# agsiddhant/PBML_Mantle_Convection

Hardware: AMD Instinct MI355X
Metric: training samples/sec (2-D 506x506 Stokes fields) (higher is better)
Workload: dtype f16+bf16; 1 GPU; CFG-3: symmetric U-Net (levels 5, c_h 16, k 5, repeats 3, reflect) + L1 data loss + divergence + Stokes momentum residual, 506x506, per-GPU batch 32, Adam, HIP-graph replay; global_batch=32, parallelism=dp1

## Files before the change

pbml_mantle_convection_amd/build_ext.py:

```python
import os
import subprocess
import sys

HERE = os.path.dirname(os.path.abspath(__file__))
CSRC = os.path.join(HERE, "csrc")
LIB = os.path.join(HERE, "libmantle_hip.so")
SOURCES = ["elementwise.hip", "conv_api.hip", "conv_f32.hip", "conv_bf16.hip", "conv_rr_bf16.hip", "loss.hip", "optim.hip"]
HEADERS = ["common.h", "conv_common.h", "conv_rr.h", os.path.join("..", "..", "include", "mantle_hip.h")]
FLAGS = ["-O3", "--offload-arch=gfx950", "-fPIC", "-std=c++17", "-Wall", "-Wno-unused-function",
         "-ffp-contract=off"]


EXTRA_FLAGS = {"conv_rr_bf16.hip": ["-fno-slp-vectorize"]}


def _stale(target, deps):
    if not os.path.exists(target):
        return True
    t = os.path.getmtime(target)
    return any(os.path.getmtime(d) > t for d in deps)


def build(force=False, verbose=True):
    hipcc = os.environ.get("HIPCC", "/opt/rocm/bin/hipcc")
    hdrs = [os.path.join(CSRC, h) for h in HEADERS]
    objdir = os.path.join(HERE, "build")
    os.makedirs(objdir, exist_ok=True)
    objs = []
    procs = []
    for src in SOURCES:
        s = os.path.join(CSRC, src)
        o = os.path.join(objdir, src.replace(".hip", ".o"))
        objs.append(o)
        if force or _stale(o, [s] + hdrs):
            cmd = [hipcc, *FLAGS, *EXTRA_FLAGS.get(src, []), "-c", s, "-o", o]
            if verbose:
                print(" ".join(cmd), flush=True)
            procs.append((src, subprocess.Popen(cmd)))
    for src, p in procs:
        if p.wait() != 0:
            raise RuntimeError(f"hipcc failed on {src}")
    if force or procs or _stale(LIB, objs):
        cmd = [hipcc, "--offload-arch=gfx950", "-shared", "-fPIC", *objs, "-o", LIB]
        if verbose:
            print(" ".join(cmd), flush=True)
        subprocess.check_call(cmd)
    return LIB


if __name__ == "__main__":
    build(force="--force" in sys.argv)
    print(LIB)
```

pbml_mantle_convection_amd/csrc/conv_api.hip:

```cpp
#include "conv_rr.h"

int mc_conv2d_f32(const ConvGeom& g, const void* x0, const void* x1, const void* bank, const float* bias, void* y0,
                  void* y1, float* part, const ConvFuse& fz, int fuse, hipStream_t s);
int mc_wgrad_f32(const ConvGeom& g, const void* x0, const void* x1, const void* dy, void* part, const ConvFuse& fz, int fuse,
                 hipStream_t s);
int mc_bf16_tile(const mc_conv_desc* d, int* th, int* tw);
size_t mc_bf16_bank_bytes(const ConvGeom& g, int dgrad);
int mc_bf16_pack(const ConvGeom& g, const float* w_unique, int dgrad, void* packed, hipStream_t s);
int mc_conv2d_bf16(const ConvGeom& g, const void* x0, const void* x1, const void* bank, const float* bias, void* y0,
                   void* y1, float* part, const ConvFuse& fz, int fuse, hipStream_t s);
int mc_wgrad_bf16(const ConvGeom& g, const void* x0, const void* x1, const void* dy, void* part, const ConvFuse& fz, int fuse,
                  hipStream_t s);
const char* mc_bf16_kernel_name(const ConvGeom& g);
void mc_bf16_bank_dims(const ConvGeom& g, int dgrad, int& chunks, int& steps, int& ntiles);
bool mc_rr_applies(int dtype, int cout, int wo, bool full_pad);
size_t mc_rr_bank_bytes(const ConvGeom& g, int dgrad);
int mc_rr_pack(const ConvGeom& g, const float* w_unique, int dgrad, void* packed, hipStream_t s);
int mc_conv2d_rr(const ConvGeom& g, const void* x0, const void* x1, const void* bank, const float* bias, void* y0, void* y1,
                 float* part, const ConvFuse& fz, int fuse, hipStream_t s);
const char* mc_rr_kernel_name(const ConvGeom& g, int fuse);

namespace {

bool rr_desc(const mc_conv_desc* d) {
  return mc_rr_applies(d->dtype, d->c_out, d->w + 2 * d->pad - d->k + 1, d->pad == d->k - 1);
}

int geom_for(const mc_conv_desc* d, ConvGeom& g) {
  if (!d) return MC_EINVAL;
  int th = 16, tw = 16;
  if (mc_is16(d->dtype)) {
    if (rr_desc(d)) { th = RR_R; tw = RR_TW; }
    else {
      int rc = mc_bf16_tile(d, &th, &tw);
      if (rc) return rc;
    }
  } else if (d->dtype != MC_F32) {
    return MC_EUNSUPPORTED;
  }
  return conv_geom(d, th, tw, g);
}
int stat_slots(const mc_conv_desc* d, const ConvGeom& g) { return rr_desc(d) ? g.tiles * RR_STRIPS : g.tiles; }

__global__ void k_pack_f32(ConvGeom g, const float* __restrict__ wu, int dgrad, float* __restrict__ bank, size_t total) {
  for (size_t i = blockIdx.x * (size_t)blockDim.x + threadIdx.x; i < total; i += (size_t)gridDim.x * blockDim.x)
    bank[i] = pack_value_f32(g, wu, i, dgrad);
}

struct PkJob {
  int K, Cout, CBin, CB0, Cin0, Cin1, Cin, U, nh, nv, nq, CBout, CinP, CoutP;
  int dgrad, steps, ntiles, bf16, f16, rr, first_block;
  unsigned total;
  const float* w;
  void* out;
};
constexpr int PK_MAX = 24;
struct PkTable { int n; PkJob j[PK_MAX]; };

__global__ void k_pack_batched(PkTable t) {
  int ji = 0;
#pragma unroll 1
  for (int k = 1; k < t.n; ++k) if ((int)blockIdx.x >= t.j[k].first_block) ji = k;
  const PkJob& job = t.j[ji];
  const int nblk = (ji + 1 < t.n ? t.j[ji + 1].first_block : (int)gridDim.x) - job.first_block;
  for (size_t i = (size_t)(blockIdx.x - job.first_block) * blockDim.x + threadIdx.x; i < job.total; i += (size_t)nblk * blockDim.x) {
    if (job.rr || job.bf16) {
      const float v = job.rr ? rr_pack_value(job, job.w, i, job.dgrad, job.ntiles)
                             : pack_value_bf16(job, job.w, i, job.dgrad, job.steps, job.ntiles);
      reinterpret_cast<bf16_t*>(job.out)[i] = job.f16 ? __builtin_bit_cast(bf16_t, (_Float16)v) : f2bf(v);
    } else {
      reinterpret_cast<float*>(job.out)[i] = pack_value_f32(job, job.w, i, job.dgrad);
    }
  }
}

struct WfJob {
  int K, U, nh, nv, nq, Cin, Cin0, CB0, CinP, CoutP, Cout, G, first_block;
  const float* part;
  float* dw;
  float* db;
};
constexpr int WF_MAX = 32;
struct WfTable { int n; WfJob j[WF_MAX]; };

constexpr int WF_WAVES = 16;
__device__ __forceinline__ void wgrad_finalize_block(const WfJob& g, int lblock) {
  const int K = g.K, KK = K * K;
  const int nch = wg_chunks(g.CinP);
  const size_t slab = wg_slab_floats(g.CoutP, g.CinP, KK);
  const size_t nW = (size_t)KK * nch * g.U * 16;
  const size_t total = nW + g.Cout;
  const int e = threadIdx.x & 63, w = threadIdx.x >> 6, NWV = (int)blockDim.x >> 6;
  const size_t i = (size_t)lblock * 64 + e;
  __shared__ float red[WF_WAVES][64];
  float s = 0.f;
  long dst = -1;
  if (i < total) {
    size_t o1, ox[3] = {0, 0, 0};
    int nx = 0;
    bool live = true;
    if (i < nW) {
      int cl = (int)(i & 15);
      size_t r = i >> 4;
      int u = (int)(r % g.U); r /= g.U;
      int chunk = (int)(r % nch);
      int tap = (int)(r / nch);
      int cip = chunk * 16 + cl;
      int ci = cip < g.CB0 * 8 ? cip : g.Cin0 + (cip - g.CB0 * 8);
      live = cip < g.CB0 * 8 ? cip < g.Cin0 : ci < g.Cin;
      int ky = tap / K, kx = tap - ky * K;
      o1 = wg_index(tap, cip, u, g.CoutP, nch);
      const int tfx = ky * K + (K - 1 - kx), tfy = (K - 1 - ky) * K + kx, tfxy = (K - 1 - ky) * K + (K - 1 - kx);
      if (u < g.nh) { nx = 1; ox[0] = wg_index(tfx, cip, g.U + u, g.CoutP, nch); }
      else if (u < g.nh + g.nv) { nx = 1; ox[0] = wg_index(tfy, cip, g.U + u, g.CoutP, nch); }
      else if (u < g.nh + g.nv + g.nq) {
        const int c0 = g.U + g.nh + g.nv + (u - g.nh - g.nv);
        nx = 3;
        ox[0] = wg_index(tfx, cip, c0, g.CoutP, nch); ox[1] = wg_index(tfy, cip, c0 + g.nq, g.CoutP, nch);
        ox[2] = wg_index(tfxy, cip, c0 + 2 * g.nq, g.CoutP, nch);
      }
      dst = ((long)u * g.Cin + ci) * KK + tap;
    } else {
      o1 = (size_t)KK * nch * g.CoutP * 16 + (i - nW);
      dst = -2 - (long)(i - nW);
    }
    if (live) {
      const float* part = g.part;
      float a0 = 0.f, a1 = 0.f, a2 = 0.f, a3 = 0.f;
      int G = w;
      for (; G + 3 * NWV < g.G; G += 4 * NWV) {
        a0 += part[(size_t)G * slab + o1]; a1 += part[(size_t)(G + NWV) * slab + o1];
        a2 += part[(size_t)(G + 2 * NWV) * slab + o1]; a3 += part[(size_t)(G + 3 * NWV) * slab + o1];
        for (int m = 0; m < nx; ++m) {
          a0 += part[(size_t)G * slab + ox[m]]; a1 += part[(size_t)(G + NWV) * slab + ox[m]];
          a2 += part[(size_t)(G + 2 * NWV) * slab + ox[m]]; a3 += part[(size_t)(G + 3 * NWV) * slab + ox[m]];
        }
      }
      for (; G < g.G; G += NWV) {
        a0 += part[(size_t)G * slab + o1];
        for (int m = 0; m < nx; ++m) a0 += part[(size_t)G * slab + ox[m]];
      }
      s = (a0 + a1) + (a2 + a3);
    } else {
      dst = -1;
    }
  }
  red[w][e] = s;
  __syncthreads();
  if (w == 0 && dst != -1) {
    float r = 0.f;
    for (int k = 0; k < NWV; k += 4) r += (red[k][e] + red[k + 1][e]) + (red[k + 2][e] + red[k + 3][e]);
    if (dst >= 0) { if (g.dw) g.dw[dst] += r; }
    else if (g.db) g.db[-2 - dst] += r;
  }
}

__global__ __launch_bounds__(64 * WF_WAVES) void k_wgrad_finalize(WfTable t) {
  int ji = 0;
#pragma unroll 1
  for (int k = 1; k < t.n; ++k) if ((int)blockIdx.x >= t.j[k].first_block) ji = k;
  wgrad_finalize_block(t.j[ji], blockIdx.x - t.j[ji].first_block);
}

int wf_fill(const mc_conv_desc* d, const void* partials, float* dw, float* db, WfJob& j, int& blocks) {
  ConvGeom g;
  int rc = geom_for(d, g);
  if (rc) return rc;
  if (!partials || (!dw && !db)) return MC_EINVAL;
  j.K = g.K; j.U = g.U; j.Cin = g.Cin; j.Cin0 = g.Cin0; j.CB0 = g.CB0; j.CinP = g.CinP; j.CoutP = g.CoutP; j.Cout = g.Cout;
  j.nh = g.nh; j.nv = g.nv; j.nq = g.nq; j.G = g.wgrad_G; j.part = (const float*)partials; j.dw = dw; j.db = db;
  size_t total = (size_t)g.K * g.K * wg_chunks(g.CinP) * g.U * 16 + g.Cout;
  blocks = (int)((total + 63) / 64);
  return MC_OK;
}

}

static bool bank_is_rr(const ConvGeom& g, int dgrad) {
  return dgrad ? mc_rr_applies(g.dtype, g.Cin, g.W + 2 * g.pad, true) : mc_rr_applies(g.dtype, g.Cout, g.Wo, g.pad == g.K - 1);
}

extern "C" {

int mc_version(void) { return 200; }

const char* mc_strerror(int code) {
  switch (code) {
    case MC_OK: return "ok";
    case MC_EINVAL: return "invalid argument or shape";
    case MC_EUNSUPPORTED: return "unsupported configuration";
    case MC_EWORKSPACE: return "workspace too small";
    default: return code > 0 ? hipGetErrorString((hipError_t)code) : "unknown error";
  }
}

size_t mc_packed_weight_bytes(const mc_conv_desc* d, int32_t dgrad) {
  ConvGeom g;
  if (geom_for(d, g)) return 0;
  if (bank_is_rr(g, dgrad)) return mc_rr_bank_bytes(g, dgrad);
  if (mc_is16(g.dtype)) return mc_bf16_bank_bytes(g, dgrad);
  int cbin = dgrad ? g.CBout : g.CBin, cop = dgrad ? g.CinP : g.CoutP;
  return (size_t)cbin * g.K * g.K * 8 * cop * sizeof(float);
}

int mc_pack_weights(const mc_conv_desc* d, const float* w_unique, int32_t dgrad, void* packed, void* stream) {
  ConvGeom g;
  int rc = geom_for(d, g);
  if (rc) return rc;
  if (!w_unique || !packed) return MC_EINVAL;
  if (bank_is_rr(g, dgrad)) return mc_rr_pack(g, w_unique, dgrad, packed, (hipStream_t)stream);
  if (mc_is16(g.dtype)) return mc_bf16_pack(g, w_unique, dgrad, packed, (hipStream_t)stream);
  size_t total = mc_packed_weight_bytes(d, dgrad) / sizeof(float);
  int blocks = (int)((total + 255) / 256);
  if (blocks > 2048) blocks = 2048;
  hipLaunchKernelGGL(k_pack_f32, dim3(blocks), dim3(256), 0, (hipStream_t)stream, g, w_unique, dgrad, (float*)packed, total);
  MC_CHECK_LAUNCH();
  return MC_OK;
}

const char* mc_conv_kernel_name(const mc_conv_desc* d) {
  ConvGeom g;
  if (geom_for(d, g)) return "unsupported";
  if (rr_desc(d)) return mc_rr_kernel_name(g, 0);
  if (mc_is16(g.dtype)) return mc_bf16_kernel_name(g);
  return g.K == 5 ? "k_conv_direct_f32<5>" : "k_conv_direct_f32<3>";
}

int32_t mc_conv_tiles(const mc_conv_desc* d) {
  ConvGeom g;
  if (geom_for(d, g)) return -1;
  return stat_slots(d, g);
}

static bool act_ok(int a) { return a >= MC_ACT_NONE && a <= MC_ACT_ELU; }

static int fill_prologue(const mc_conv_prologue* pro, ConvFuse& fz, int& rc) {
  rc = MC_OK;
  if (!pro) return 0;
  if (!act_ok(pro->act0) || !act_ok(pro->act1)) { rc = MC_EINVAL; return 0; }
  fz.coef0 = pro->coef0; fz.coef1 = pro->coef1; fz.act0 = pro->act0; fz.act1 = pro->act1;
  return (pro->coef0 || pro->coef1 || pro->act0 != MC_ACT_NONE || pro->act1 != MC_ACT_NONE) ? 1 : 0;
}

int mc_conv2d_fused(const mc_conv_desc* d, const void* x0, const void* x1, const mc_conv_prologue* pro,
                    const void* packed_w, const float* bias, void* y0, void* y1, float* stat_partials,
                    const mc_conv_epilogue* epi, void* stream) {
  ConvGeom g;
  int rc = geom_for(d, g);
  if (rc) return rc;
  if (!x0 || !packed_w || !y0 || (g.Cin1 > 0 && !x1) || (g.split8 > 0 && !y1)) return MC_EINVAL;
  ConvFuse fz = conv_fuse_none();
  int fuse = fill_prologue(pro, fz, rc);
  if (rc) return rc;
  if (epi) {
    if (fuse) return MC_EUNSUPPORTED;
    if (!epi->y || !epi->partials || !act_ok(epi->act) || epi->pad < 0 || epi->hs <= 0 || epi->ws <= 0) return MC_EINVAL;
    if (epi->pad_mode < MC_PAD_ZEROS || epi->pad_mode > MC_PAD_REFLECT) return MC_EINVAL;
    if (g.split8 > 0 || stat_partials || g.out_f32) return MC_EUNSUPPORTED;
    if (g.Ho != epi->hs + 2 * epi->pad || g.Wo != epi->ws + 2 * epi->pad) return MC_EINVAL;
    fz.ey = epi->y; fz.ecoef = epi->coef; fz.epart = epi->partials; fz.eact = epi->act; fz.epad = epi->pad;
    fz.ezero = epi->pad_mode == MC_PAD_ZEROS || epi->pad == 0; fz.ehs = epi->hs; fz.ews = epi->ws;
    if (epi->y_f16 && g.dtype != MC_BF16) return MC_EINVAL;
    fz.ey16 = epi->y_f16 ? 1 : 0;
    if (epi->part_stride < stat_slots(d, g)) return MC_EINVAL;
    fz.estride = epi->part_stride;
    fuse = 2;
  }
  if (rr_desc(d)) return mc_conv2d_rr(g, x0, x1, packed_w, bias, y0, y1, stat_partials, fz, fuse, (hipStream_t)stream);
  if (mc_is16(g.dtype)) return mc_conv2d_bf16(g, x0, x1, packed_w, bias, y0, y1, stat_partials, fz, fuse, (hipStream_t)stream);
  return mc_conv2d_f32(g, x0, x1, packed_w, bias, y0, y1, stat_partials, fz, fuse, (hipStream_t)stream);
}

int mc_conv2d(const mc_conv_desc* d, const void* x0, const void* x1, const void* packed_w, const float* bias, void* y0,
              void* y1, float* stat_partials, void* stream) {
  return mc_conv2d_fused(d, x0, x1, nullptr, packed_w, bias, y0, y1, stat_partials, nullptr, stream);
}

size_t mc_conv_bank_read_extent(const mc_conv_desc* d) {
  ConvGeom g;
  if (geom_for(d, g)) return 0;
  const int KK = g.K * g.K;
  if (rr_desc(d)) {
    const size_t nfrag = g.K == 5 ? RR<5>::NFRAG : RR<3>::NFRAG;
    const size_t chunks = (g.CBin + 1) / 2, groups = (g.Cout + 15) / 16;
    return (((chunks - 1) * groups + (groups - 1)) * nfrag * 64 + (nfrag * 64 - 1)) * 16 + 16;
  }
  if (mc_is16(g.dtype)) {
    int chunks, steps, ntiles;
    mc_bf16_bank_dims(g, 0, chunks, steps, ntiles);
    const size_t last = ((size_t)(chunks - 1) * steps + (steps - 1)) * ntiles + (ntiles - 1);
    return (last * 64 + 63) * 16 + 16;
  }
  const int ncog = (g.CoutP + 15) / 16, co0 = 16 * (ncog - 1);
  const int comax = g.CoutP - 1 - co0;
  const size_t last = (((size_t)(g.CBin - 1) * KK + (KK - 1)) * 8 + 7) * g.CoutP + co0 + (comax >= 15 ? 15 : comax);
  return (last + 1) * sizeof(float);
}

size_t mc_wgrad_partial_bytes(const mc_conv_desc* d) {
  ConvGeom g;
  if (geom_for(d, g)) return 0;
  return (size_t)g.wgrad_G * wg_slab_floats(g.CoutP, g.CinP, g.K * g.K) * sizeof(float);
}

int mc_conv2d_wgrad_fused(const mc_conv_desc* d, const void* x0, const void* x1, const mc_conv_prologue* pro,
                          const void* dy, void* partials, void* stream) {
  ConvGeom g;
  int rc = geom_for(d, g);
  if (rc) return rc;
  if (!x0 || !dy || !partials || (g.Cin1 > 0 && !x1)) return MC_EINVAL;
  ConvFuse fz = conv_fuse_none();
  const int fuse = fill_prologue(pro, fz, rc);
  if (rc) return rc;
  if (mc_is16(g.dtype)) return mc_wgrad_bf16(g, x0, x1, dy, partials, fz, fuse, (hipStream_t)stream);
  return mc_wgrad_f32(g, x0, x1, dy, partials, fz, fuse, (hipStream_t)stream);
}

int mc_conv2d_wgrad(const mc_conv_desc* d, const void* x0, const void* x1, const void* dy, void* partials,
                    void* stream) {
  return mc_conv2d_wgrad_fused(d, x0, x1, nullptr, dy, partials, stream);
}

int mc_conv2d_wgrad_finalize_batched(const mc_conv_desc* descs, const void* const* partials, float* const* dw,
                                     float* const* db, int32_t n, void* stream) {
  if (!descs || !partials || !dw || !db || n <= 0) return MC_EINVAL;
  for (int pass = 0; pass < 2; ++pass) {
    WfTable t;
    t.n = 0;
    int blocks = 0;
    auto flush = [&]() {
      if (t.n == 0) return;
      hipLaunchKernelGGL(k_wgrad_finalize, dim3(blocks), dim3(pass == 0 ? 64 * WF_WAVES : 256), 0, (hipStream_t)stream, t);
      t.n = 0; blocks = 0;
    };
    for (int k = 0; k < n; ++k) {
      WfJob j;
      int b = 0;
      int rc = wf_fill(&descs[k], partials[k], dw[k], db[k], j, b);
      if (rc) return rc;
      if ((j.G >= 128) != (pass == 0)) continue;
      j.first_block = blocks;
      t.j[t.n++] = j;
      blocks += b;
      if (t.n == WF_MAX) flush();
    }
    flush();
    MC_CHECK_LAUNCH();
  }
  return MC_OK;
}

int mc_conv2d_wgrad_finalize(const mc_conv_desc* d, const void* partials, float* dw_unique, float* dbias,
                             void* stream) {
  return mc_conv2d_wgrad_finalize_batched(d, &partials, &dw_unique, &dbias, 1, stream);
}

int mc_pack_weights_batched(const mc_conv_desc* descs, const float* const* w_unique, const int32_t* dgrad,
                            void* const* packed, int32_t n, void* stream) {
  if (!descs || !w_unique || !dgrad || !packed || n <= 0) return MC_EINVAL;
  for (int base = 0; base < n; base += PK_MAX) {
    PkTable t;
    t.n = n - base < PK_MAX ? n - base : PK_MAX;
    int blocks = 0;
    for (int k = 0; k < t.n; ++k) {
      ConvGeom g;
      int rc = geom_for(&descs[base + k], g);
      if (rc) return rc;
      if (!w_unique[base + k] || !packed[base + k]) return MC_EINVAL;
      PkJob& j = t.j[k];
      j.K = g.K; j.Cout = g.Cout; j.CBin = g.CBin; j.CB0 = g.CB0; j.Cin0 = g.Cin0; j.Cin1 = g.Cin1; j.Cin = g.Cin; j.U = g.U;
      j.nh = g.nh; j.nv = g.nv; j.nq = g.nq;
      j.CBout = g.CBout; j.CinP = g.CinP; j.CoutP = g.CoutP; j.dgrad = dgrad[base + k]; j.bf16 = mc_is16(g.dtype);
      j.f16 = (g.dtype == MC_MIX16 && !j.dgrad) ? 1 : 0;
      j.rr = bank_is_rr(g, j.dgrad);
      size_t total;
      if (j.rr) {
        j.steps = 0;
        j.ntiles = ((j.dgrad ? g.CinP : g.Cout) + 15) / 16;
        total = mc_rr_bank_bytes(g, j.dgrad) / 2;
      } else if (j.bf16) {
        int chunks;
        mc_bf16_bank_dims(g, j.dgrad, chunks, j.steps, j.ntiles);
        total = (size_t)chunks * j.steps * j.ntiles * 64 * 8;
      } else {
        j.steps = 0; j.ntiles = 0;
        total = (size_t)(j.dgrad ? g.CBout : g.CBin) * g.K * g.K * 8 * (j.dgrad ? g.CinP : g.CoutP);
      }
      j.total = (unsigned)total;
      j.w = w_unique[base + k];
      j.out = packed[base + k];
      j.first_block = blocks;
      int b = (int)((total + 256 * 8 - 1) / (256 * 8));
      blocks += b < 1 ? 1 : b;
    }
    hipLaunchKernelGGL(k_pack_batched, dim3(blocks), dim3(256), 0, (hipStream_t)stream, t);
    MC_CHECK_LAUNCH();
  }
  return MC_OK;
}

}
```

Measured before the change: 3235 samples/s.

## Add flat-plane MFMA conv kernel for deep low-resolution 5x5 bf16/f16 layers

Adds a new persistent MFMA convolution kernel for 16-bit 5x5 full-padded convolutions whose padded row width fits in a fixed limit. These are the deep, small-spatial U-Net levels that previously went through the generic tiled bf16 path. The kernel stages a whole flattened padded plane strip into LDS and walks output positions linearly, with XCD-aware block remapping, register double-buffered fragments and fused prologue/epilogue/stat reductions. It is on by default behind an env switch. It adds code complexity and depends on the weight bank layout matching the existing bf16 packer.

```diff
diff --git a/pbml_mantle_convection_amd/build_ext.py b/pbml_mantle_convection_amd/build_ext.py
--- a/pbml_mantle_convection_amd/build_ext.py
+++ b/pbml_mantle_convection_amd/build_ext.py
@@ -5,7 +5,7 @@
 HERE = os.path.dirname(os.path.abspath(__file__))
 CSRC = os.path.join(HERE, "csrc")
 LIB = os.path.join(HERE, "libmantle_hip.so")
-SOURCES = ["elementwise.hip", "conv_api.hip", "conv_f32.hip", "conv_bf16.hip", "conv_rr_bf16.hip", "loss.hip", "optim.hip"]
+SOURCES = ["elementwise.hip", "conv_api.hip", "conv_f32.hip", "conv_bf16.hip", "conv_flat_bf16.hip", "conv_rr_bf16.hip", "loss.hip", "optim.hip"]
 HEADERS = ["common.h", "conv_common.h", "conv_rr.h", os.path.join("..", "..", "include", "mantle_hip.h")]
 FLAGS = ["-O3", "--offload-arch=gfx950", "-fPIC", "-std=c++17", "-Wall", "-Wno-unused-function",
          "-ffp-contract=off"]
diff --git a/pbml_mantle_convection_amd/csrc/conv_api.hip b/pbml_mantle_convection_amd/csrc/conv_api.hip
--- a/pbml_mantle_convection_amd/csrc/conv_api.hip
+++ b/pbml_mantle_convection_amd/csrc/conv_api.hip
@@ -19,26 +19,40 @@
 int mc_conv2d_rr(const ConvGeom& g, const void* x0, const void* x1, const void* bank, const float* bias, void* y0, void* y1,
                  float* part, const ConvFuse& fz, int fuse, hipStream_t s);
 const char* mc_rr_kernel_name(const ConvGeom& g, int fuse);
+bool mc_flat_fits(int c_out, int k, int wo);
+int mc_flat_items(const ConvGeom& g);
+const char* mc_flat_kernel_name(const ConvGeom& g);
+int mc_conv2d_flat(const ConvGeom& g, const void* x0, const void* x1, const void* bank, const float* bias, void* y0, void* y1,
+                   float* part, const ConvFuse& fz, int fuse, hipStream_t s);
 
 namespace {
 
 bool rr_desc(const mc_conv_desc* d) {
   return mc_rr_applies(d->dtype, d->c_out, d->w + 2 * d->pad - d->k + 1, d->pad == d->k - 1);
+}
+
+bool flat_desc(const mc_conv_desc* d) {
+  static const int on = getenv("MC_CONV_DEEP") ? atoi(getenv("MC_CONV_DEEP")) : 1;
+  return on && mc_is16(d->dtype) && !d->out_f32 && d->pad == d->k - 1 && !rr_desc(d) &&
+         mc_flat_fits(d->c_out, d->k, d->w + 2 * d->pad - d->k + 1);
 }
 
 int geom_for(const mc_conv_desc* d, ConvGeom& g) {
   if (!d) return MC_EINVAL;
   int th = 16, tw = 16;
+  const bool flat = mc_is16(d->dtype) && flat_desc(d);
   if (mc_is16(d->dtype)) {
     if (rr_desc(d)) { th = RR_R; tw = RR_TW; }
-    else {
+    else if (!flat) {
       int rc = mc_bf16_tile(d, &th, &tw);
       if (rc) return rc;
     }
   } else if (d->dtype != MC_F32) {
     return MC_EUNSUPPORTED;
   }
-  return conv_geom(d, th, tw, g);
+  int rc = conv_geom(d, th, tw, g);
+  if (rc == MC_OK && flat) { g.tiles = mc_flat_items(g); g.tiles_x = g.tiles; g.tiles_y = 1; }
+  return rc;
 }
 int stat_slots(const mc_conv_desc* d, const ConvGeom& g) { return rr_desc(d) ? g.tiles * RR_STRIPS : g.tiles; }
 
@@ -222,6 +236,7 @@
   ConvGeom g;
   if (geom_for(d, g)) return "unsupported";
   if (rr_desc(d)) return mc_rr_kernel_name(g, 0);
+  if (flat_desc(d)) return mc_flat_kernel_name(g);
   if (mc_is16(g.dtype)) return mc_bf16_kernel_name(g);
   return g.K == 5 ? "k_conv_direct_f32<5>" : "k_conv_direct_f32<3>";
 }
@@ -267,6 +282,7 @@
     fuse = 2;
   }
   if (rr_desc(d)) return mc_conv2d_rr(g, x0, x1, packed_w, bias, y0, y1, stat_partials, fz, fuse, (hipStream_t)stream);
+  if (flat_desc(d)) return mc_conv2d_flat(g, x0, x1, packed_w, bias, y0, y1, stat_partials, fz, fuse, (hipStream_t)stream);
   if (mc_is16(g.dtype)) return mc_conv2d_bf16(g, x0, x1, packed_w, bias, y0, y1, stat_partials, fz, fuse, (hipStream_t)stream);
   return mc_conv2d_f32(g, x0, x1, packed_w, bias, y0, y1, stat_partials, fz, fuse, (hipStream_t)stream);
 }
diff --git a/pbml_mantle_convection_amd/csrc/conv_flat_bf16.hip b/pbml_mantle_convection_amd/csrc/conv_flat_bf16.hip
--- /dev/null
+++ b/pbml_mantle_convection_amd/csrc/conv_flat_bf16.hip
@@ -0,0 +1,373 @@
+#include "conv_common.h"
+#include <type_traits>
+
+using bf16x8 = __attribute__((ext_vector_type(8))) short;
+using f16x8 = __attribute__((ext_vector_type(8))) _Float16;
+using f32x4 = __attribute__((ext_vector_type(4))) float;
+typedef unsigned int v4u __attribute__((ext_vector_type(4)));
+
+namespace {
+
+constexpr int FL_K = 5;
+constexpr int FL_STEPS = (FL_K * FL_K * 2 + 3) / 4;
+constexpr int FL_WAVES = 4, FL_NTHR = 64 * FL_WAVES;
+constexpr int FL_PMAX = 140;
+
+__host__ __device__ constexpr int fl_plane(int mtiles, int P) { return (mtiles * 16 + (FL_K - 1) * P + (FL_K - 1) + 15) / 16 * 16; }
+
+__device__ __forceinline__ int fl_xcd_remap(int bid, int nwg) {
+  const int xcd = bid & 7, q = nwg >> 3, r = nwg & 7;
+  return (xcd < r ? xcd * (q + 1) : r * (q + 1) + (xcd - r) * q) + (bid >> 3);
+}
+
+template <bool H16> __device__ __forceinline__ f32x4 fl_mfma(bf16x8 a, bf16x8 b, f32x4 c) {
+  if constexpr (H16) return __builtin_amdgcn_mfma_f32_16x16x32_f16(__builtin_bit_cast(f16x8, a), __builtin_bit_cast(f16x8, b), c, 0, 0, 0);
+  else return __builtin_amdgcn_mfma_f32_16x16x32_bf16(a, b, c, 0, 0, 0);
+}
+
+template <int MTW, int NTW, int WN, int FUSE, bool H16>
+__global__ __launch_bounds__(FL_NTHR, 2) void k_conv_flat_mfma(ConvGeom g, const bf16_t* __restrict__ x0,
+                                                            const bf16_t* __restrict__ x1, const bf16_t* __restrict__ bank,
+                                                            const float* __restrict__ bias, bf16_t* __restrict__ y0,
+                                                            bf16_t* __restrict__ y1, float* __restrict__ part, int ipi,
+                                                            ConvFuse fz) {
+  constexpr int NT = NTW * WN;
+  constexpr int WROWS = FL_WAVES / WN;
+  constexpr int MTILES = MTW * WROWS;
+  constexpr int POS = MTILES * 16;
+  constexpr int PER = (fl_plane(MTILES, FL_PMAX) + FL_NTHR - 1) / FL_NTHR;
+  extern __shared__ uint4 fl_lds[];
+  __shared__ float red[FL_WAVES][NT * 16 * 2];
+
+  const int P = g.Wo + FL_K - 1;
+  const int PLANE = fl_plane(MTILES, P);
+  uint4* in_s = fl_lds;
+
+  const int grp = blockIdx.y;
+  const int bid = fl_xcd_remap(blockIdx.x, gridDim.x);
+  const int lane = threadIdx.x & 63, wave = __builtin_amdgcn_readfirstlane(threadIdx.x >> 6);
+  const int m = lane & 15, gq = lane >> 4;
+  const int ntile0 = grp * NT;
+  const int wm = wave / WN, nt_w0 = (wave % WN) * NTW;
+  const int ntiles_total = gridDim.y * NT;
+  const int chunks = (g.CBin + 1) / 2;
+  const int items = g.N * ipi;
+  const int my_items = (items - bid + (int)gridDim.x - 1) / (int)gridDim.x;
+  const int total_stages = my_items * chunks;
+  const int HP = g.Ho + FL_K - 1;
+
+  unsigned soff[PER];
+  unsigned okm = 0xffffffffu;
+  int cur_item = -1;
+  auto slot_offsets = [&](int wi) {
+    const int n = wi / ipi, it0 = wi - n * ipi;
+    const int q0 = it0 * POS;
+    okm = 0xffffffffu;
+#pragma unroll
+    for (int it = 0; it < PER; ++it) {
+      const int i = (int)threadIdx.x + it * FL_NTHR;
+      const int f = q0 + i;
+      const int r = f / P, c = f - r * P;
+      bool oky, okx;
+      const int sy = pad_map_sel(r - g.pad, g.H, g.pad_mode, oky);
+      const int sx = pad_map_sel(c - g.pad, g.W, g.pad_mode, okx);
+      const bool ok = oky && okx && r < HP && i < PLANE;
+      soff[it] = ok ? (unsigned)(sy * g.W + sx) * 16u : 0xFFFFFFF0u;
+      if (!ok) okm &= ~(1u << it);
+    }
+  };
+
+  v4u rin[2][PER];
+  float psc[2][8], psh[2][8];
+  int pact[2] = {-1, -1};
+  auto prefetch = [&](int t) {
+    const int jitem = t / chunks, ck = t - jitem * chunks;
+    const int wi = bid + jitem * (int)gridDim.x;
+    if (wi != cur_item) { slot_offsets(wi); cur_item = wi; }
+    const int n = wi / ipi;
+#pragma unroll
+    for (int cb = 0; cb < 2; ++cb) {
+      const int gcb = ck * 2 + cb;
+      const int gcc = min(gcb, g.CBin - 1);
+      const bool second = gcc >= g.CB0;
+      const int scb = second ? gcc - g.CB0 : gcc;
+      const int sC8 = second ? g.CB1 : g.CB0;
+      const size_t plane_bytes = (size_t)g.H * g.W * 16;
+      const char* pbase = reinterpret_cast<const char*>(second ? x1 : x0) + ((size_t)n * sC8 + scb) * plane_bytes;
+      __amdgpu_buffer_rsrc_t rs = __builtin_amdgcn_make_buffer_rsrc((void*)pbase, 0, gcb < g.CBin ? (int)plane_bytes : 0, 0x00020000);
+      if constexpr (FUSE == 1) {
+        const float* ct = second ? fz.coef1 : fz.coef0;
+        const int a = second ? fz.act1 : fz.act0;
+        pact[cb] = (gcb < g.CBin && (ct != nullptr || a != MC_ACT_NONE)) ? a : -1;
+        if (pact[cb] >= 0) load_coef8(ct, n, sC8 * 8, scb, psc[cb], psh[cb]);
+      }
+#pragma unroll
+      for (int it = 0; it < PER; ++it) rin[cb][it] = __builtin_amdgcn_raw_buffer_load_b128(rs, soff[it], 0, 0);
+    }
+  };
+  auto commit = [&]() {
+#pragma unroll
+    for (int cb = 0; cb < 2; ++cb) {
+#pragma unroll
+      for (int it = 0; it < PER; ++it) {
+        const int i = (int)threadIdx.x + it * FL_NTHR;
+        if (i >= PLANE) continue;
+        uint4 v = make_uint4(rin[cb][it][0], rin[cb][it][1], rin[cb][it][2], rin[cb][it][3]);
+        if (FUSE == 1 && pact[cb] >= 0) {
+          v = H16 ? xform_f16x8(v, psc[cb], psh[cb], pact[cb]) : xform_bf16x8(v, psc[cb], psh[cb], pact[cb]);
+          if (!((okm >> it) & 1u)) v = make_uint4(0, 0, 0, 0);
+        }
+        in_s[cb * PLANE + i] = v;
+      }
+    }
+  };
+
+  float bv[NTW][4];
+#pragma unroll
+  for (int tt = 0; tt < NTW; ++tt)
+#pragma unroll
+    for (int r = 0; r < 4; ++r) {
+      const int co = (ntile0 + nt_w0 + tt) * 16 + gq * 4 + r;
+      bv[tt][r] = (bias && co < g.Cout) ? bias[co] : 0.f;
+    }
+
+  f32x4 acc[MTW][NTW];
+  for (int t = 0; t < total_stages; ++t) {
+    const int jitem = t / chunks, ck = t - jitem * chunks;
+    if (ck == 0) {
+#pragma unroll
+      for (int i = 0; i < MTW; ++i)
+#pragma unroll
+        for (int tt = 0; tt < NTW; ++tt) acc[i][tt] = (f32x4){bv[tt][0], bv[tt][1], bv[tt][2], bv[tt][3]};
+    }
+    prefetch(t);
+    __syncthreads();
+    commit();
+    __syncthreads();
+    const uint4* wglob = reinterpret_cast<const uint4*>(bank) + ((size_t)ck * FL_STEPS * ntiles_total + ntile0 + nt_w0) * 64 + lane;
+    const int abase = (gq & 1) * PLANE + wm * MTW * 16 + m;
+    int kx = gq >> 1, ky = 0;
+    auto load_frags = [&](int sidx, bf16x8 (&xf)[MTW], bf16x8 (&wf)[NTW]) {
+      const bool dummy = ky >= FL_K;
+      const uint4* ap = in_s + abase + (dummy ? 0 : ky * P + kx);
+      kx += 2;
+      if (kx >= FL_K) { kx -= FL_K; ky += 1; }
+#pragma unroll
+      for (int tt = 0; tt < NTW; ++tt) wf[tt] = __builtin_bit_cast(bf16x8, wglob[((size_t)sidx * ntiles_total + tt) * 64]);
+#pragma unroll
+      for (int i = 0; i < MTW; ++i) xf[i] = *reinterpret_cast<const bf16x8*>(ap + i * 16);
+    };
+    bf16x8 xr[2][MTW], wr[2][NTW];
+    load_frags(0, xr[0], wr[0]);
+#pragma unroll
+    for (int s = 0; s < FL_STEPS; ++s) {
+      if (s + 1 < FL_STEPS) load_frags(s + 1, xr[(s + 1) & 1], wr[(s + 1) & 1]);
+      __builtin_amdgcn_sched_barrier(0);
+#pragma unroll
+      for (int i = 0; i < MTW; ++i)
+#pragma unroll
+        for (int tt = 0; tt < NTW; ++tt) acc[i][tt] = fl_mfma<(H16 && FUSE != 2)>(wr[s & 1][tt], xr[s & 1][i], acc[i][tt]);
+      __builtin_amdgcn_sched_barrier(0);
+    }
+    if (ck != chunks - 1) continue;
+
+    const int wi = bid + jitem * (int)gridDim.x;
+    const int n = wi / ipi, item = wi - n * ipi;
+    const int q0 = item * POS + wm * MTW * 16 + m;
+    int oyv[MTW], oxv[MTW];
+#pragma unroll
+    for (int i = 0; i < MTW; ++i) {
+      const int q = q0 + i * 16;
+      oyv[i] = q / P; oxv[i] = q - oyv[i] * P;
+    }
+    f32x2 s1[NTW][2], s2[NTW][2];
+#pragma unroll
+    for (int tt = 0; tt < NTW; ++tt)
+#pragma unroll
+      for (int h = 0; h < 2; ++h) { s1[tt][h] = (f32x2){0.f, 0.f}; s2[tt][h] = (f32x2){0.f, 0.f}; }
+    bf16_t* dstb[NTW];
+    bool cobok[NTW];
+    int cbcv[NTW];
+    const int C8o = g.split8 > 0 ? g.split8 : g.CBout;
+#pragma unroll
+    for (int tt = 0; tt < NTW; ++tt) {
+      const int cob = (ntile0 + nt_w0 + tt) * 2 + (gq >> 1);
+      cobok[tt] = cob < g.CBout;
+      const int cbc = min(cob, g.CBout - 1);
+      cbcv[tt] = cbc;
+      if (g.split8 > 0 && cbc >= g.split8) dstb[tt] = y1 + cb8_index(n, cbc - g.split8, 0, 0, g.CBout - g.split8, g.Ho, g.Wo) + (gq & 1) * 4;
+      else dstb[tt] = y0 + cb8_index(n, cbc, 0, 0, C8o, g.Ho, g.Wo) + (gq & 1) * 4;
+    }
+    if constexpr (FUSE != 2) {
+#pragma unroll
+      for (int i = 0; i < MTW; ++i) {
+        const bool inb = oyv[i] < g.Ho && oxv[i] < g.Wo;
+        const size_t off = ((size_t)oyv[i] * g.Wo + oxv[i]) * 8;
+#pragma unroll
+        for (int tt = 0; tt < NTW; ++tt) {
+          const f32x2 v01 = (f32x2){acc[i][tt][0], acc[i][tt][1]}, v23 = (f32x2){acc[i][tt][2], acc[i][tt][3]};
+          if (inb) {
+            s1[tt][0] += v01; s1[tt][1] += v23;
+            s2[tt][0] = pk_fma(v01, v01, s2[tt][0]); s2[tt][1] = pk_fma(v23, v23, s2[tt][1]);
+            if (cobok[tt]) {
+              uint2 pk;
+              if constexpr (H16) { pk.x = pk_f16(v01.x, v01.y); pk.y = pk_f16(v23.x, v23.y); }
+              else { pk.x = pk_bf16(v01.x, v01.y); pk.y = pk_bf16(v23.x, v23.y); }
+              *reinterpret_cast<uint2*>(dstb[tt] + off) = pk;
+            }
+          }
+        }
+      }
+    } else {
+      const int p = fz.epad, fr = fz.ezero ? 0 : p + 1;
+      const bf16_t* ey = reinterpret_cast<const bf16_t*>(fz.ey);
+#pragma unroll
+      for (int tt = 0; tt < NTW; ++tt) {
+        const int cbc = cbcv[tt];
+        float csc[4], csh[4], cme[4], crs[4];
+#pragma unroll
+        for (int r = 0; r < 4; ++r) {
+          if (fz.ecoef) {
+            const float4 c4 = reinterpret_cast<const float4*>(fz.ecoef)[(size_t)n * g.CoutP + cbc * 8 + (gq & 1) * 4 + r];
+            csc[r] = c4.x; csh[r] = c4.y; cme[r] = c4.z; crs[r] = c4.w;
+          } else { csc[r] = 1.f; csh[r] = 0.f; cme[r] = 0.f; crs[r] = 0.f; }
+        }
+#pragma unroll
+        for (int i = 0; i < MTW; ++i) {
+          const int iy = oyv[i] - p, ix = oxv[i] - p;
+          const bool fin = cobok[tt] && iy >= fr && iy < fz.ehs - fr && ix >= fr && ix < fz.ews - fr;
+          const int cy = min(max(iy, 0), fz.ehs - 1), cx = min(max(ix, 0), fz.ews - 1);
+          const uint2 yv = *reinterpret_cast<const uint2*>(ey + cb8_index(n, cbc, cy, cx, g.CBout, fz.ehs, fz.ews) + (gq & 1) * 4);
+          const bool inb = oyv[i] < g.Ho && oxv[i] < g.Wo;
+          const size_t off = ((size_t)oyv[i] * g.Wo + oxv[i]) * 8;
+          float yf[4];
+          if constexpr (H16) {
+            const f32x2 ya = unpk_f16(yv.x), yb = unpk_f16(yv.y);
+            yf[0] = ya.x; yf[1] = ya.y; yf[2] = yb.x; yf[3] = yb.y;
+          } else {
+            yf[0] = __uint_as_float(yv.x << 16); yf[1] = __uint_as_float(yv.x & 0xffff0000u);
+            yf[2] = __uint_as_float(yv.y << 16); yf[3] = __uint_as_float(yv.y & 0xffff0000u);
+          }
+          float o[4];
+#pragma unroll
+          for (int h = 0; h < 2; ++h) {
+            const f32x2 yy = (f32x2){yf[2 * h], yf[2 * h + 1]};
+            const f32x2 z = pk_fma(yy, (f32x2){csc[2 * h], csc[2 * h + 1]}, (f32x2){csh[2 * h], csh[2 * h + 1]});
+            f32x2 gp;
+            if (fz.eact == MC_ACT_GELU) gp = gelu_grad_poly2(z);
+            else gp = (f32x2){act_bwd(z.x, fz.eact), act_bwd(z.y, fz.eact)};
+            const f32x2 da = (f32x2){acc[i][tt][2 * h], acc[i][tt][2 * h + 1]};
+            const f32x2 dz = da * gp;
+            const f32x2 yh = (yy - (f32x2){cme[2 * h], cme[2 * h + 1]}) * (f32x2){crs[2 * h], crs[2 * h + 1]};
+            if (fin && inb) { s1[tt][h] += dz; s2[tt][h] = pk_fma(dz, yh, s2[tt][h]); }
+            o[2 * h] = fin ? dz.x : da.x; o[2 * h + 1] = fin ? dz.y : da.y;
+          }
+          if (inb && cobok[tt]) {
+            uint2 pk;
+            pk.x = (uint32_t)f2bf(o[0]) | ((uint32_t)f2bf(o[1]) << 16);
+            pk.y = (uint32_t)f2bf(o[2]) | ((uint32_t)f2bf(o[3]) << 16);
+            *reinterpret_cast<uint2*>(dstb[tt] + off) = pk;
+          }
+        }
+      }
+    }
+    float* pp = FUSE == 2 ? fz.epart : part;
+    if (pp) {
+#pragma unroll
+      for (int tt = 0; tt < NTW; ++tt) {
+        float q8[8] = {s1[tt][0].x, s2[tt][0].x, s1[tt][0].y, s2[tt][0].y, s1[tt][1].x, s2[tt][1].x, s1[tt][1].y, s2[tt][1].y};
+        const bool b3 = m & 8, b2 = m & 4, b1 = m & 2;
+        float q4[4], q2[2], q1;
+#pragma unroll
+        for (int k = 0; k < 4; ++k) q4[k] = (b3 ? q8[4 + k] : q8[k]) + __shfl_xor(b3 ? q8[k] : q8[4 + k], 8, 64);
+#pragma unroll
+        for (int k = 0; k < 2; ++k) q2[k] = (b2 ? q4[2 + k] : q4[k]) + __shfl_xor(b2 ? q4[k] : q4[2 + k], 4, 64);
+        q1 = (b1 ? q2[1] : q2[0]) + __shfl_xor(b1 ? q2[0] : q2[1], 2, 64);
+        q1 += __shfl_xor(q1, 1, 64);
+        if ((m & 1) == 0) red[wave][((nt_w0 + tt) * 16 + gq * 4) * 2 + (m >> 1)] = q1;
+      }
+      __syncthreads();
+      if (threadIdx.x < NT * 32) {
+        const int co = ntile0 * 16 + (threadIdx.x >> 1);
+        if (co < g.CoutP) {
+          float r = 0.f;
+#pragma unroll
+          for (int wv = 0; wv < WROWS; ++wv) r += red[wv * WN + (int)(threadIdx.x >> 5) / NTW][threadIdx.x];
+          pp[(((size_t)n * (FUSE == 2 ? fz.estride : ipi) + item) * g.CoutP + co) * 2 + (threadIdx.x & 1)] = r;
+        }
+      }
+    }
+  }
+}
+
+struct FlCfg { int mtw, ntw, wn; };
+constexpr FlCfg FL_CFGS[] = {{8, 2, 2}, {4, 2, 2}, {8, 2, 1}, {4, 2, 1}};
+constexpr int FL_NCFG = sizeof(FL_CFGS) / sizeof(FL_CFGS[0]);
+
+inline int fl_mtiles(const FlCfg& c) { return c.mtw * (FL_WAVES / c.wn); }
+
+int fl_cfg_index(int nt, int ho, int P) {
+  static const int forced = getenv("MC_CONV_DEEP_CFG") ? atoi(getenv("MC_CONV_DEEP_CFG")) : -1;
+  if (forced >= 0 && forced < FL_NCFG && FL_CFGS[forced].ntw * FL_CFGS[forced].wn == nt) return forced;
+  const long pos = (long)ho * P;
+  if (nt == 2) return pos >= 8192 ? 2 : 3;
+  return pos >= 2048 ? 0 : 1;
+}
+
+}
+
+bool mc_flat_fits(int c_out, int k, int wo) {
+  const int nt = (c_out + 15) / 16;
+  return k == FL_K && nt >= 2 && nt % 2 == 0 && wo + FL_K - 1 <= FL_PMAX;
+}
+
+int mc_flat_items(const ConvGeom& g) {
+  const int nt = (g.Cout + 15) / 16;
+  const int npb = nt % 4 == 0 ? 4 : 2;
+  const int P = g.Wo + FL_K - 1;
+  const int pos = fl_mtiles(FL_CFGS[fl_cfg_index(npb, g.Ho, P)]) * 16;
+  return (g.Ho * P + pos - 1) / pos;
+}
+
+const char* mc_flat_kernel_name(const ConvGeom& g) {
+  const int nt = (g.Cout + 15) / 16;
+  static const char* names[FL_NCFG] = {"k_conv_flat_mfma<8,2,2>", "k_conv_flat_mfma<4,2,2>", "k_conv_flat_mfma<8,2,1>",
+                                       "k_conv_flat_mfma<4,2,1>"};
+  return names[fl_cfg_index(nt % 4 == 0 ? 4 : 2, g.Ho, g.Wo + FL_K - 1)];
+}
+
+int mc_conv2d_flat(const ConvGeom& g, const void* x0, const void* x1, const void* bank, const float* bias, void* y0,
+                   void* y1, float* part, const ConvFuse& fz, int fuse, hipStream_t s) {
+  if (g.K != FL_K || g.out_f32 || !mc_flat_fits(g.Cout, g.K, g.Wo)) return MC_EUNSUPPORTED;
+  const int nt_total = (g.Cout + 15) / 16;
+  const int npb = nt_total % 4 == 0 ? 4 : 2;
+  const int P = g.Wo + FL_K - 1;
+  const int ci = fl_cfg_index(npb, g.Ho, P);
+  const FlCfg c = FL_CFGS[ci];
+  const int ipi = mc_flat_items(g);
+  const int groups = nt_total / npb;
+  const int items = g.N * ipi;
+  static const int cap_total = getenv("MC_CONV_CAP") ? atoi(getenv("MC_CONV_CAP")) : 4096;
+  const int cap = cap_total / groups > 0 ? cap_total / groups : 1;
+  dim3 grid(items < cap ? items : cap, groups, 1);
+  const size_t lds = (size_t)2 * fl_plane(fl_mtiles(c), P) * 16;
+  const bool h16 = fuse == 2 ? fz.ey16 != 0 : g.dtype == MC_MIX16;
+#define FL_LAUNCH_H(MTW, NTW, WN, FU, H)                                                                                  \
+  hipLaunchKernelGGL((k_conv_flat_mfma<MTW, NTW, WN, FU, H>), grid, dim3(FL_NTHR), lds, s, g, (const bf16_t*)x0,          \
+                     (const bf16_t*)x1, (const bf16_t*)bank, bias, (bf16_t*)y0, (bf16_t*)y1, part, ipi, fz)
+#define FL_LAUNCH_F(MTW, NTW, WN, FU) do { if (h16) FL_LAUNCH_H(MTW, NTW, WN, FU, true); else FL_LAUNCH_H(MTW, NTW, WN, FU, false); } while (0)
+#define FL_LAUNCH(MTW, NTW, WN)                                                                                           \
+  do { if (fuse == 0) FL_LAUNCH_F(MTW, NTW, WN, 0); else if (fuse == 1) FL_LAUNCH_F(MTW, NTW, WN, 1);                     \
+       else FL_LAUNCH_F(MTW, NTW, WN, 2); } while (0)
+  switch (ci) {
+    case 0: FL_LAUNCH(8, 2, 2); break;
+    case 1: FL_LAUNCH(4, 2, 2); break;
+    case 2: FL_LAUNCH(8, 2, 1); break;
+    default: FL_LAUNCH(4, 2, 1); break;
+  }
+#undef FL_LAUNCH
+#undef FL_LAUNCH_F
+#undef FL_LAUNCH_H
+  MC_CHECK_LAUNCH();
+  return MC_OK;
+}
```

Result: no change. 3250 samples/s, median of 6 (+0.5%).
